# 2235854410/CCVPE

Hardware: AMD Instinct MI355X
Metric: query images/sec (VIGOR, 512x512 sat / 320x640 grd) (higher is better)
Workload: dtype f32; 1 GPU; vigor_samearea_fov360_b32; variant=vigor_ori_prior, batch_per_gpu=32, global_batch=32, parallelism=image-parallel x1, all_gather of 20 B/query results, schedule=two streams per GPU (aerial encoder + orientation decoder on the second)

## Files before the change

ccvpe_amd/csrc/kernels.h:

```cpp
#pragma once
#include <functional>
#include <vector>
#include <hip/hip_runtime.h>
#include <stdint.h>
#include "ticket.h"

namespace ccvpe {

extern thread_local unsigned long long g_launches;
#define CCVPE_LAUNCH(...) do { ++::ccvpe::g_launches; hipLaunchKernelGGL(__VA_ARGS__); } while (0)

struct LdsAttr { size_t set[16] = {0}; };
inline void ensure_dynamic_lds(LdsAttr& state, const void* kernel, size_t bytes) {
    int dev = 0;
    if (hipGetDevice(&dev) != hipSuccess || dev < 0 || dev >= 16) dev = 0;
    if (bytes > state.set[dev] && hipFuncSetAttribute(kernel, hipFuncAttributeMaxDynamicSharedMemorySize, (int)bytes) == hipSuccess) state.set[dev] = bytes;
}

enum Act { ACT_NONE = 0, ACT_RELU = 1, ACT_SWISH = 2 };

struct Dst {
    float* ptr;
    int ld;
    int coff;
    int split;
    long long plane;
};

enum { MODE_CONV = 0, MODE_DECONV = 1 };

struct ConvParams {
    const float* in;
    int in_ld;
    int B, H, W, Cin;
    int OH, OW;
    int KH, KW, stride, pad_t, pad_l;
    const float* wpk;
    const unsigned short* w_hi;
    const unsigned short* w_lo;
    int Kpad;
    int Npad;
    int nchunks;
    const float* bias;
    int N;
    int act;
    const float* gate;
    const float* resid;
    int resid_ld;
    Dst dst[3];
    int ndst;
    int mode;
    int deconv_cout;
    int M;
    unsigned in_bytes;
    int in_split;
    unsigned in_plane_bytes;
    unsigned w_plane_bytes;
    unsigned gate_bytes;
    int taps4;
    int kfull_chunks;
    int kfull_c0;
    int knc;
    int div_4t_mul;
    int div_nc_mul;
    int div_kw_mul;
    int vec_epi;
    int splitk;
    float* partial;
    size_t partial_floats;
    unsigned* tickets;
    int split_fused;
    unsigned fdw_mul, fdw_shift, fdh_mul, fdh_shift;
    const float* wino_w;
    int wino_n16;
    int wino_nb, wino_n16_off;
    unsigned wino_bytes;
    const float* wino4_w;
    unsigned wino4_bytes;
    const float* wino4x_w;
    unsigned wino4x_bytes;
    int wino4x_cfg;
    const float* proj_w;
    unsigned proj_bytes;
    const float* se_rows;
    int se_nrows, se_sq;
    float se_inv_hw;
    const float* se_b1;
    const float* se_w2;
    const float* se_b2;
};

enum { TILE_AUTO = 0 };
static constexpr int CONV_TICKETS = 8192;
static constexpr int SPLIT_FUSED = 64;
int conv_igemm_num_tiles();
double conv_igemm_tile_util(const ConvParams& p, int tile);
long long conv_igemm_tile_blocks(const ConvParams& p, int tile);
int conv_igemm_prepare(ConvParams& p);
int conv_igemm_k_index(int cin, int taps, int tap, int c);
int launch_conv_igemm(const ConvParams& p, int tile, hipStream_t s);
int conv_igemm_npad();
bool conv_igemm_tile_is_bf16x3(int tile);
bool conv_igemm_tile_can_fuse_split(int tile);
void launch_splitk_reduce(const ConvParams& p, hipStream_t s);
struct Bf16x3Tile { int bm, bn; const char* name; void (*launch)(const ConvParams&, hipStream_t); };
int bf16x3_num_tiles();
const Bf16x3Tile* bf16x3_tile(int i);
struct WinoTile { int bm, bn; const char* name; void (*launch)(const ConvParams&, hipStream_t); int f; int xcfg; };
int wino_num_tiles();
const WinoTile* wino_tile(int i);
bool conv_wino_supported(const ConvParams& p);
bool conv_wino4_supported(const ConvParams& p);
bool conv_wino_tile_supported(const ConvParams& p, int tile);
bool conv_igemm_tile_is_wino4(int tile);
void launch_wino4_64(const ConvParams& p, hipStream_t s);
void launch_wino4_128(const ConvParams& p, hipStream_t s);
bool conv_wino4_tail_applied();
bool conv_igemm_tile_is_wino4x(int tile);
int conv_igemm_tile_wino4x_cfg(int tile);
void launch_wino4x(const ConvParams& p, hipStream_t s);
bool conv_wino4x_supported(const ConvParams& p);
int conv_wino4x_config(int N);
size_t conv_wino4x_pack(int N, int cin, const std::function<float(int, int, int)>& get, std::vector<float>& out, int* cfg_out);
size_t conv_wino4_pack(int N, int cin, const std::function<float(int, int, int)>& get, std::vector<float>& out);
bool conv_igemm_tile_is_wino(int tile);
size_t conv_wino_pack(int N, int cin, const std::function<float(int, int, int)>& get, std::vector<float>& out, int* n16_out);
struct PwTile { int bm, bn; const char* name; void (*launch)(const ConvParams&, hipStream_t); int proj_rt; };
int pw_num_tiles();
const PwTile* pw_tile(int i);
bool conv_pw_supported(const ConvParams& p);
bool conv_pw_fits(int bn, int kpad);
bool conv_pw_tile_ok(int i, const ConvParams& p);
int conv_pw_tile_proj_rt(int i);
int conv_igemm_tile_proj_rt(int tile);
int conv_proj_lat_tile();
bool conv_proj_supported(const ConvParams& p, int rt);
void launch_proj(const ConvParams& p, int rt, hipStream_t s);
bool conv_proj_wanted(int N, int cin);
bool conv_proj_has(int rt, int N);
size_t conv_proj_pack(int N, int cin, const std::function<float(int, int)>& get, std::vector<float>& out, int taps = 1);
bool conv_proj_lat_wanted(int taps, int KH, int KW, int cinp);
bool conv_igemm_tile_is_pw(int tile);
bool conv_igemm_tile_is_proj(int tile);
int conv_igemm_last_tile();
const char* conv_igemm_tile_name(int tile);

struct StemParams {
    const float* in;
    int B, H, W, OH, OW;
    int pad_t, pad_l;
    int circular;
    const float* w;
    const float* bias;
    float* out;
};
void launch_stem(const StemParams& p, hipStream_t s);

struct StemDwParams {
    StemParams st;
    const float* wd;
    const float* bd;
    float* out;
    float* pool_partial;
    SeTicket se;
};
int stem_dw_tiles(int OH, int OW);
void launch_stem_dw(const StemDwParams& p, hipStream_t s);

struct DwParams {
    const float* in;
    int B, H, W, C, OH, OW;
    int k, stride, pad_t, pad_l, circular;
    const float* w;
    const float* bias;
    float* out;
    float* pool_partial;
    int S;
    SeTicket se;
};
void launch_depthwise(const DwParams& p, hipStream_t s);
int depthwise_strip_lanes(int B, int OH, int OW, int C, int k, int stride);

struct MbFrontParams {
    const float* x;
    int B, H, W, Cin, cinp;
    int mid;
    const float* we;
    const float* be;
    const float* wd;
    const float* bd;
    int k, s, pad_t, pad_l, circular, OH, OW;
    float* out;
    float* pool;
    SeTicket se;
    int spread;
};
void launch_mbconv_front(const MbFrontParams& p, hipStream_t s);
int mbconv_front_tiles(int k, int s, int OH, int OW);
int mbconv_front_ticket_rows(const MbFrontParams& p);
int mbconv_image_ticket_rows(const MbFrontParams& p);
int mbconv_front_ticket_split(const MbFrontParams& p);
bool mbconv_front_supported(int k, int s, int cin, int mid);
bool mbconv_front_profitable(int k);
bool mbconv_image_supported(const MbFrontParams& p);
int mbconv_image_strips(const MbFrontParams& p);
void launch_mbconv_image(const MbFrontParams& p, hipStream_t s);

struct SeParams {
    const float* pool_partial;
    int B, S, C, SQ;
    float inv_hw;
    const float* w1;
    const float* b1;
    const float* w2;
    const float* b2;
    float* gate;
    float* pooled;
    int SC;
    float* sq;
};
void launch_se(const SeParams& p, hipStream_t s);

struct GrdDescParams {
    const float* y;
    int B, Hf, Wf, Ntot;
    int nlev;
    int c[6], off[6];
    const float* wh[6];
    float b2[6];
    float* desc;
    int loff[6];
    int Ltot;
};
void launch_grd_desc(const GrdDescParams& p, hipStream_t s);

struct MatchParams {
    const float* x;
    int x_ld;
    int B, HW, C;
    const float* g;
    int g_ld, L;
    int R;
    int shift[32];
    uint32_t inmax;
    float* ms;
    float* cat_max;  int cat_max_ld;
    float* cat_all;  int cat_all_ld;  int rpad;
    int P;
    float* gg_scratch;
    int prep_done;
    int no_wide;
};
void launch_match(const MatchParams& p, hipStream_t s);
void launch_match_prep(const MatchParams& p, hipStream_t s);
void launch_match_prep_all(const MatchParams* ps, int n, hipStream_t s);
int match_pixels_per_block(int HW, int C);
size_t match_scratch_floats(int C);

struct TailConvParams {
    const float* in;
    int B, H, W;
    const float* w;
    float bias[2];
    int cout;
    int normalize;
    float* out;
    float* raw;
};
void launch_tail_conv(const TailConvParams& p, hipStream_t s);
// ... 138 lines not shown
```

ccvpe_amd/csrc/kernels_wino.hip:

```cpp
#include "igemm_common.h"

#include <algorithm>

namespace ccvpe {

typedef float f32x2 __attribute__((ext_vector_type(2)));

#ifndef CCVPE_WINO_SCALAR_COLUMNS
#define CCVPE_WINO_SCALAR_COLUMNS 0
#endif

template <int NW, int NM, int GC, bool FUSED = false>
__global__ __launch_bounds__(NW * NM * 64) __attribute__((amdgpu_waves_per_eu(2, 2))) void conv_wino_kernel(const ConvParams p) {
    constexpr int NT = NW * NM * 64;
    constexpr int NITEM = 256 * NM;
    constexpr int ITEMS = (NITEM + NT - 1) / NT;
    constexpr int PXS = GC * 8 + 4;
    constexpr int PROWS = 8 * NM + 2;
    constexpr int RAW_F4 = PROWS * 18 * GC * 2;
    constexpr int RAW_ITEMS = (RAW_F4 + NT - 1) / NT;
    constexpr unsigned OOB = 0x80000000u;
    constexpr bool VDB = NM == 1;
    constexpr int VSZ = 4096 * NM;

// ... 163 lines not shown
                    for (int x = 0; x < 16; ++x) Vw[x * 256 + g_lds[i]] = vi[x];
                }
            }
            __syncthreads();
            if (!VDB) {
#pragma unroll
                for (int i = 0; i < ITEMS; ++i)
                    if (NT * ITEMS == NITEM || tid + i * NT < NITEM) {
#pragma unroll
                        for (int x = 0; x < 16; ++x) Vw[x * 256 + g_lds[i]] = v[VDB ? 0 : i][x];
                    }
            }
            const bool group_end = sub == glen - 1;
            if (group_end) {
                CCVPE_WINO_STORE_RAW();
                gstart += glen;
                ++gidx;
                glen = glen_lo + (gidx < n_hi ? 1 : 0);
            }
            if (!VDB || group_end) __syncthreads();
            vbuf ^= 1;
            const unsigned wb = last_chunk ? w_base_n : w_base;
            const int chn = last_chunk ? c_begin : ch + 1;
            __builtin_amdgcn_sched_barrier(0);
            f32x2 fa[2][2][2];
#define CCVPE_WINO_FRAGS(buf, g)                                                                         \
    _Pragma("unroll") for (int e = 0; e < 2; ++e) {                                                      \
        fa[buf][e][0] = *reinterpret_cast<const f32x2*>(va + ((g) * 2 + e) * 256);                       \
        fa[buf][e][1] = *reinterpret_cast<const f32x2*>(va + ((g) * 2 + e) * 256 + 128);                 \
    }
            CCVPE_WINO_FRAGS(0, 0);
#pragma unroll
            for (int g = 0; g < 8; ++g) {
                const int cur = g & 1;
                if (g + 1 < 8) { CCVPE_WINO_FRAGS(cur ^ 1, g + 1); }
                __builtin_amdgcn_sched_barrier(0);
#pragma unroll
                for (int e = 0; e < 2; ++e) {
                    const int x = g * 2 + e;
                    acc[x][0] = __builtin_amdgcn_mfma_f32_16x16x4f32(bq[x].x, fa[cur][e][0].x, acc[x][0], 0, 0, 0);
                    acc[x][1] = __builtin_amdgcn_mfma_f32_16x16x4f32(bq[x].x, fa[cur][e][1].x, acc[x][1], 0, 0, 0);
                    acc[x][0] = __builtin_amdgcn_mfma_f32_16x16x4f32(bq[x].y, fa[cur][e][0].y, acc[x][0], 0, 0, 0);
                    acc[x][1] = __builtin_amdgcn_mfma_f32_16x16x4f32(bq[x].y, fa[cur][e][1].y, acc[x][1], 0, 0, 0);
                }
                __builtin_amdgcn_sched_barrier(0);
                CCVPE_WINO_LOAD_B(wb, chn, g);
            }
#undef CCVPE_WINO_FRAGS
            __builtin_amdgcn_sched_barrier(0);
        }

        {
            const int n = (nb * NW + wave) * 16 + 4 * (lane >> 4);
            f32x4 bias = {0.f, 0.f, 0.f, 0.f};
            if (!split) {
#pragma unroll
                for (int i = 0; i < 4; ++i) bias[i] = n + i < p.N ? p.bias[n + i] : 0.f;
            }
            const float lo = act == ACT_RELU ? 0.f : -__builtin_inff();
            const size_t pix0 = ((size_t)b * p.H + (size_t)(by * NM + wset) * 8) * p.W + (size_t)bx * 16;
            float* obase = split ? p.partial + ((size_t)blockIdx.z * p.M + pix0) * p.N : p.dst[0].ptr + pix0 * ld + p.dst[0].coff;
            const __amdgpu_buffer_rsrc_t o_rsrc = __builtin_amdgcn_make_buffer_rsrc(obase, 0, 0x7fffffff, 0x00020000);
            const int tl = lane & 15;
            const unsigned o_lane = n < p.N ? (unsigned)((((tl >> 3) * 2 * p.W + (tl & 7) * 2) * ld + n) * 4) : OOB;
#pragma unroll
            for (int h = 0; h < 2; ++h) {
                f32x4 tt[2][4];
#pragma unroll
                for (int c = 0; c < 4; ++c) {
                    tt[0][c] = acc[0 * 4 + c][h] + acc[1 * 4 + c][h] + acc[2 * 4 + c][h];
                    tt[1][c] = acc[1 * 4 + c][h] - acc[2 * 4 + c][h] - acc[3 * 4 + c][h];
                }
#pragma unroll
                for (int a = 0; a < 2; ++a) {
                    f32x4 y[2];
                    y[0] = tt[a][0] + tt[a][1] + tt[a][2] + bias;
                    y[1] = tt[a][1] - tt[a][2] - tt[a][3] + bias;
#pragma unroll
                    for (int dx = 0; dx < 2; ++dx) {
                        f32x4 v;
#pragma unroll
                        for (int i = 0; i < 4; ++i) v[i] = y[dx][i] < lo ? lo : y[dx][i];
                        const int soff = (((h * 4 + a) * p.W + dx) * ld) * 4;
                        __builtin_amdgcn_raw_buffer_store_b128(__builtin_bit_cast(__attribute__((__vector_size__(4 * sizeof(unsigned)))) unsigned, v), o_rsrc, o_lane, soff, FUSED ? 16 : 0);
                        __builtin_amdgcn_sched_barrier(0);
                        asm volatile("s_nop 1");
                        __builtin_amdgcn_sched_barrier(0);
                    }
                }
            }
        }
        if (FUSED) {
            if (splitk_ticket(p, item, reinterpret_cast<unsigned*>(Vs))) fin_mask |= 1ull << ordinal;
        }
        if (FUSED) ++ordinal;
        if (!have_n) break;
#pragma unroll
        for (int x = 0; x < 16; ++x) {
            acc[x][0] = f32x4{0.f, 0.f, 0.f, 0.f};
            acc[x][1] = f32x4{0.f, 0.f, 0.f, 0.f};
        }
        item = item_n; nb = nb_n; b = b_n; by = by_n; bx = bx_n; w_base = w_base_n;
    }
    while (FUSED && fin_mask) {
        const int k = __builtin_ctzll(fin_mask);
        fin_mask &= fin_mask - 1;
        int nb_f, b_f, by_f, bx_f;
        CCVPE_WINO_DECODE(item_first + k * stride, nb_f, b_f, by_f, bx_f);
        splitk_finish<NT>(p, (b_f * p.H + by_f * NM * 8) * p.W + bx_f * 16, 8 * NM, 16, p.W, nb_f * NW * 16, NW * 16);
    }
#undef CCVPE_WINO_LOAD_RAW
#undef CCVPE_WINO_STORE_RAW
#undef CCVPE_WINO_LOAD_B
#undef CCVPE_WINO_ROFF
#undef CCVPE_WINO_DECODE
#undef CCVPE_WINO_WBASE
}

template <int NW, int NM, int GC>
static void launch_wino(const ConvParams& p_in, hipStream_t s) {
    ConvParams p = p_in;
    if (p.splitk > 1) {
        const int nch = p.Cin >> 3;
        const int per = (nch + p.splitk - 1) / p.splitk;
        p.splitk = (nch + per - 1) / per;
    }
    constexpr size_t lds = (4096 * NM * (NM == 1 ? 2 : 1) + (8 * NM + 2) * 18 * (GC * 8 + 4)) * sizeof(float);
    static_assert(2 * lds <= 160 * 1024, "two workgroups per CU");
    static LdsAttr attr, attr_f;
    const int mblocks = p.B * (p.W >> 4) * (p.H / (8 * NM));
    const int nblocks = (p.wino_n16 + NW - 1) / NW;
    const int resident = 2 * 256 / (p.splitk > 1 ? p.splitk : 1);
    dim3 grid(std::min(mblocks * nblocks, std::max(resident, 8)), 1, p.splitk > 1 ? p.splitk : 1);
    if (p.splitk <= 1 || p.tickets == nullptr || mblocks * nblocks > CONV_TICKETS || (mblocks * nblocks + (int)grid.x - 1) / (int)grid.x + 1 > 64) p.split_fused = 0;
    if (p.split_fused) {
        auto kern = conv_wino_kernel<NW, NM, GC, true>;
        ensure_dynamic_lds(attr_f, reinterpret_cast<const void*>(kern), lds);
        CCVPE_LAUNCH(kern, grid, dim3(NW * NM * 64), lds, s, p);
        return;
    }
    auto kern = conv_wino_kernel<NW, NM, GC, false>;
    ensure_dynamic_lds(attr, reinterpret_cast<const void*>(kern), lds);
    CCVPE_LAUNCH(kern, grid, dim3(NW * NM * 64), lds, s, p);
    if (p.splitk > 1) launch_splitk_reduce(p, s);
}

static const WinoTile WINO_TILES[] = {
    {256, 32, "conv_wino_64x32", launch_wino<2, 2, 2>, 2, -1},
    {128, 48, "conv_wino_32x48", launch_wino<3, 1, 2>, 2, -1},
    {128, 64, "conv_wino_32x64", launch_wino<4, 1, 4>, 2, -1},
    {128, 80, "conv_wino_32x80", launch_wino<5, 1, 4>, 2, -1},
    {256, 48, "conv_wino_64x48", launch_wino<3, 2, 2>, 2, -1},
    {256, 64, "conv_wino4_16x64", launch_wino4_64, 4, -1},
    {256, 128, "conv_wino4_16x128", launch_wino4_128, 4, -1},
    {256, 32, "conv_wino4x_32", launch_wino4x, 4, 0},
    {256, 48, "conv_wino4x_48", launch_wino4x, 4, 1},
    {256, 64, "conv_wino4x_64", launch_wino4x, 4, 2},
    {256, 80, "conv_wino4x_80", launch_wino4x, 4, 3},
    {256, 96, "conv_wino4x_96", launch_wino4x, 4, 4},
    {256, 128, "conv_wino4x_128", launch_wino4x, 4, 5},
};
int wino_num_tiles() { return (int)(sizeof(WINO_TILES) / sizeof(WINO_TILES[0])); }
const WinoTile* wino_tile(int i) { return &WINO_TILES[i]; }

bool conv_wino_supported(const ConvParams& p) {
    return p.wino_w != nullptr && p.KH == 3 && p.KW == 3 && p.stride == 1 && p.pad_t == 1 && p.pad_l == 1 && p.mode == MODE_CONV &&
           p.gate == nullptr && p.resid == nullptr && p.ndst == 1 && !p.dst[0].split && !p.in_split && p.OH == p.H && p.OW == p.W &&
           p.W % 16 == 0 && p.H % 16 == 0 && p.Cin % 8 == 0 && p.N % 4 == 0 && p.dst[0].ld % 4 == 0 && p.dst[0].coff % 4 == 0;
}

size_t conv_wino_pack(int N, int cin, const std::function<float(int, int, int)>& get, std::vector<float>& out, int* n16_out) {
    static const double G[4][3] = {{1.0, 0.0, 0.0}, {0.5, 0.5, 0.5}, {0.5, -0.5, 0.5}, {0.0, 0.0, 1.0}};
    const int n16 = (N + 15) / 16;
    const int nch = cin / 8;
    out.assign((size_t)nch * 16 * n16 * 128, 0.f);
    for (int n = 0; n < N; ++n)
        for (int c = 0; c < cin; ++c) {
            double g[3][3], tmp[4][3];
            for (int i = 0; i < 3; ++i)
                for (int j = 0; j < 3; ++j) g[i][j] = (double)get(n, i * 3 + j, c);
            for (int r = 0; r < 4; ++r)
                for (int j = 0; j < 3; ++j) tmp[r][j] = G[r][0] * g[0][j] + G[r][1] * g[1][j] + G[r][2] * g[2][j];
            const int chunk = c / 8, k = c % 8;
            for (int r = 0; r < 4; ++r)
                for (int q = 0; q < 4; ++q) {
                    const double uv = tmp[r][0] * G[q][0] + tmp[r][1] * G[q][1] + tmp[r][2] * G[q][2];
                    const int xi = r * 4 + q;
                    const size_t idx = ((((size_t)chunk * 8 + xi / 2) * n16 + n / 16) * 64 + (k & 3) * 16 + (n % 16)) * 4 + (xi & 1) * 2 + (k >> 2);
                    out[idx] = (float)uv;
                }
        }
    *n16_out = n16;
    return out.size();
}

}
```

ccvpe_amd/csrc/kernels_wino4.hip:

```cpp
#include "igemm_common.h"

#include <algorithm>
#include <thread>
#include <type_traits>

namespace ccvpe {

typedef float f32x2 __attribute__((ext_vector_type(2)));

static constexpr int W4_PITCH = 20;
static constexpr int W4_PLANE = 385;
static constexpr int W4_GCH = 16;
static constexpr int W4_VFLOATS = 4 * 18 * 64 * 2;
static constexpr int W4_RAW_F4 = 18 * 18 * 4;

__device__ __forceinline__ void w4_bt(const float d0, const float d1, const float d2, const float d3, const float d4, const float d5,
                                      float& t0, float& t1, float& t2, float& t3, float& t4, float& t5) {
    const float a = fmaf(-4.f, d2, d4), b = fmaf(-4.f, d1, d3);
    const float c = d4 - d2, e = d3 - d1;
    t0 = fmaf(4.f, d0, fmaf(-5.f, d2, d4));
    t1 = a + b;
    t2 = a - b;
    t3 = fmaf(2.f, e, c);
    t4 = fmaf(-2.f, e, c);
    t5 = fmaf(4.f, d1, fmaf(-5.f, d3, d5));
}
__device__ __forceinline__ void w4_at(const float m0, const float m1, const float m2, const float m3, const float m4, const float m5,
                                      float& y0, float& y1, float& y2, float& y3) {
    const float s1 = m1 + m2, d1 = m1 - m2, s2 = m3 + m4, d2 = m3 - m4;
    y0 = m0 + s1 + s2;
    y1 = fmaf(2.f, d2, d1);
    y2 = fmaf(4.f, s2, s1);
    y3 = fmaf(8.f, d2, d1) + m5;
}

template <int NW, bool FUSED = false>
__global__ __launch_bounds__(NW * 64) __attribute__((amdgpu_waves_per_eu(2, 2))) void conv_wino4_kernel(const ConvParams p) {
    static_assert(NW == 4 || NW == 8, "waves w and w + 4 share the k-step w & 3 of a 16-channel group");
    constexpr int NT = NW * 64;
    constexpr int RAW_ITEMS = NW == 4 ? 6 : 3;
    constexpr int RAW_HALVES = RAW_ITEMS / 3;
    constexpr unsigned OOB = 0x80000000u;

    extern __shared__ __attribute__((aligned(16))) float smem[];
    float* Vs = smem;
    float* Rs = smem + W4_VFLOATS;

    const int tid = threadIdx.x;
    const int lane = tid & 63;
    const int wave = tid >> 6;

    const int mbx = p.W >> 4, mby = p.H >> 4;
    const int mblocks = p.B * mbx * mby;
    const int total = mblocks * (p.wino_nb ? p.wino_nb : (p.wino_n16 + NW - 1) / NW);

    const int xcd = blockIdx.x & 7;
    const int stride = ((int)gridDim.x >> 3) + (xcd < ((int)gridDim.x & 7) ? 1 : 0);
    const int S = p.splitk > 1 ? p.splitk : 1;
    const int item_begin = xcd * (total >> 3) + min(xcd, total & 7);
    const int item_end = item_begin + (total >> 3) + (xcd < (total & 7) ? 1 : 0);
    int item = item_begin + ((int)blockIdx.x >> 3);
    if (item >= item_end) return;
    const int item_first = item;
    int ordinal = 0;
    unsigned long long fin_mask = 0;

    const __amdgpu_buffer_rsrc_t in_rsrc = __builtin_amdgcn_make_buffer_rsrc(const_cast<float*>(p.in), 0, p.in_bytes, 0x00020000);
    const __amdgpu_buffer_rsrc_t w_rsrc = __builtin_amdgcn_make_buffer_rsrc(const_cast<float*>(p.wino4_w), 0, p.wino4_bytes, 0x00020000);

    int nb, b, by, bx;
    const int z = (int)blockIdx.z;
#define CCVPE_W4_DECODE(it_, nb_, b_, by_, bx_)                                                          \
    {                                                                                                    \
        nb_ = (it_) / mblocks;                                                                           \
        const int mb_ = (it_) - nb_ * mblocks;                                                           \
        b_ = mb_ / (mbx * mby);                                                                          \
        const int rem_ = mb_ - b_ * (mbx * mby);                                                         \
        by_ = rem_ / mbx;                                                                                \
        bx_ = rem_ - by_ * mbx;                                                                          \
    }
    CCVPE_W4_DECODE(item, nb, b, by, bx);

    unsigned r_off[RAW_ITEMS];
    const int r_ch = (tid & 3) * 4;
    const int r_px0 = tid >> 2;
#define CCVPE_W4_ROFF(b_, by_, bx_, live_)                                                               \
    _Pragma("unroll") for (int i = 0; i < RAW_ITEMS; ++i) {                                              \
        int j = tid + i * NT;                                                                            \
        asm volatile("" : "+v"(j));    \
        const int px = j >> 2, q = j & 3;                                                                \
        const int py = px / 18, pxx = px - py * 18;                                                      \
        const int y = (by_) * 16 - 1 + py, x = (bx_) * 16 - 1 + pxx;                                     \
        const bool ok = (live_) && j < W4_RAW_F4 && (unsigned)y < (unsigned)p.H && (unsigned)x < (unsigned)p.W; \
        r_off[i] = ok ? (unsigned)(((((b_) * p.H + y) * p.W + x) * p.in_ld + q * 4) * 4) : OOB;          \
    }
    CCVPE_W4_ROFF(b, by, bx, true);

    const int tk = lane & 3, ttx = (lane >> 2) & 3, tty = lane >> 4;
    const int tks = wave & 3;
    const float* t_src = Rs + (4 * tks + tk) * W4_PLANE + (4 * tty) * W4_PITCH + 4 * ttx;
    float* t_dst = Vs + ((tks * 18) * 64 + tk * 16 + tty * 4 + ttx) * 2;

    const unsigned w_quad_b = (unsigned)p.wino_n16 * 1024u;
    const unsigned w_step_b = w_quad_b * 9u;
#define CCVPE_W4_WBASE(nb_) ((nb_) * NW + wave + p.wino_n16_off < p.wino_n16 ? (unsigned)((nb_) * NW + wave + p.wino_n16_off) * 1024u + (unsigned)lane * 16u : OOB)
    unsigned w_base = CCVPE_W4_WBASE(nb);

    const int ngr_all = (p.Cin + W4_GCH - 1) / W4_GCH;
    const int g_per = (ngr_all + S - 1) / S;
    const int g_begin = min(z * g_per, ngr_all), g_end = min(g_begin + g_per, ngr_all);
    if (g_begin >= g_end) return;
    const int tail_ks = (p.Cin - (ngr_all - 1) * W4_GCH + 3) >> 2;

    f32x4 raw[3];
    float bq[36];
#define CCVPE_W4_LOAD_RAW(c0, half)                                        \
    _Pragma("unroll") for (int i = 0; i < 3; ++i) {                                                    \
        const unsigned o_ = ((c0) + r_ch < p.Cin) ? r_off[3 * (half) + i] : OOB;                         \
        raw[i] = __builtin_bit_cast(f32x4, __builtin_amdgcn_raw_buffer_load_b128(in_rsrc, o_, (c0) * 4, 0)); \
    }
#define CCVPE_W4_STORE_RAW(half)                                                                         \
    _Pragma("unroll") for (int i = 0; i < 3; ++i) {                                                    \
        const int px_ = r_px0 + (NT / 4) * (3 * (half) + i);                                             \
        if (px_ < 18 * 18) {                                                                             \
            const int py_ = (px_ * 3641) >> 16;                          \
            float* d_ = Rs + r_ch * W4_PLANE + py_ * W4_PITCH + (px_ - py_ * 18);                        \
            d_[0] = raw[i].x; d_[W4_PLANE] = raw[i].y; d_[2 * W4_PLANE] = raw[i].z; d_[3 * W4_PLANE] = raw[i].w; \
        }                                                                                                \
    }
#define CCVPE_W4_LOAD_B(wb, ks, qd)              \
    {                                                                                                    \
        const f32x4 t4_ = __builtin_bit_cast(f32x4, __builtin_amdgcn_raw_buffer_load_b128(w_rsrc, wb, (ks) * w_step_b + (qd) * w_quad_b, 0)); \
        bq[4 * (qd)] = t4_.x; bq[4 * (qd) + 1] = t4_.y; bq[4 * (qd) + 2] = t4_.z; bq[4 * (qd) + 3] = t4_.w; \
    }

    f32x4 acc[36];
#pragma unroll
    for (int x = 0; x < 36; ++x) acc[x] = f32x4{0.f, 0.f, 0.f, 0.f};

    CCVPE_W4_LOAD_RAW(g_begin * W4_GCH, 0);
#pragma unroll
    for (int qd = 0; qd < 9; ++qd) { CCVPE_W4_LOAD_B(w_base, g_begin * 4, qd); }
    CCVPE_W4_STORE_RAW(0);
    if (RAW_HALVES == 2) {
        CCVPE_W4_LOAD_RAW(g_begin * W4_GCH, 1);
        CCVPE_W4_STORE_RAW(1);
    }
    __syncthreads();

    const float* va0 = Vs + lane * 2;
    const bool split = p.splitk > 1;
    const int ld = split ? p.N : p.dst[0].ld;
    const int act = split ? ACT_NONE : p.act;

    while (true) {
        const int item_n = item + stride;
        const bool have_n = item_n < item_end;
        int nb_n, b_n, by_n, bx_n;
        CCVPE_W4_DECODE(have_n ? item_n : item, nb_n, b_n, by_n, bx_n);
        const unsigned w_base_n = have_n ? CCVPE_W4_WBASE(nb_n) : OOB;

        for (int g = g_begin; g < g_end; ++g) {
            const bool last_group = g == g_end - 1;
            const int nks = g == ngr_all - 1 ? tail_ks : 4;
            auto half_item = [&](auto hfc) {
                constexpr int HF = decltype(hfc)::value;
                float t[3][6];
                float dc[2][6];
#pragma unroll
                for (int r = 0; r < 6; ++r) dc[0][r] = t_src[r * W4_PITCH];
#pragma unroll
                for (int c = 0; c < 6; ++c) {
                    if (c + 1 < 6) {
#pragma unroll
                        for (int r = 0; r < 6; ++r) dc[(c + 1) & 1][r] = t_src[r * W4_PITCH + c + 1];
                    }
                    float u0, u1, u2, u3, u4, u5;
                    w4_bt(dc[c & 1][0], dc[c & 1][1], dc[c & 1][2], dc[c & 1][3], dc[c & 1][4], dc[c & 1][5], u0, u1, u2, u3, u4, u5);
                    t[0][c] = HF ? u3 : u0; t[1][c] = HF ? u4 : u1; t[2][c] = HF ? u5 : u2;
                }
#pragma unroll
                for (int ii = 0; ii < 3; ++ii) {
                    float v0, v1, v2, v3, v4, v5;
                    w4_bt(t[ii][0], t[ii][1], t[ii][2], t[ii][3], t[ii][4], t[ii][5], v0, v1, v2, v3, v4, v5);
                    float* td = t_dst + HF * (9 * 128) + ii * (3 * 128);
                    *reinterpret_cast<f32x2*>(td) = f32x2{v0, v1};
                    *reinterpret_cast<f32x2*>(td + 128) = f32x2{v2, v3};
                    *reinterpret_cast<f32x2*>(td + 256) = f32x2{v4, v5};
                }
            };
            if (tks >= nks) {
            } else if (NW == 4) {
                half_item(std::integral_constant<int, 0>{});
                half_item(std::integral_constant<int, 1>{});
            } else if (wave < 4) {
                half_item(std::integral_constant<int, 0>{});
            } else {
                half_item(std::integral_constant<int, 1>{});
            }
            __syncthreads();
            const int c0n = last_group ? g_begin * W4_GCH : (g + 1) * W4_GCH;
            if (last_group) { CCVPE_W4_ROFF(b_n, by_n, bx_n, have_n); }
            CCVPE_W4_LOAD_RAW(c0n, 0);
            __builtin_amdgcn_sched_barrier(0);
#pragma unroll 1
            for (int ks = 0; ks < nks; ++ks) {
                const bool last_step = last_group && ks == nks - 1;
                const unsigned wb = last_step ? w_base_n : w_base;
                const int ksn = last_step ? g_begin * 4 : g * 4 + ks + 1;
                const float* va = va0 + ks * (18 * 128);
                f32x2 fa[3];
                fa[0] = *reinterpret_cast<const f32x2*>(va);
                fa[1] = *reinterpret_cast<const f32x2*>(va + 128);
#pragma unroll
                for (int xp = 0; xp < 18; ++xp) {
                    if (xp + 2 < 18) fa[(xp + 2) % 3] = *reinterpret_cast<const f32x2*>(va + (xp + 2) * 128);
                    __builtin_amdgcn_sched_barrier(0);
                    acc[2 * xp] = __builtin_amdgcn_mfma_f32_16x16x4f32(bq[2 * xp], fa[xp % 3].x, acc[2 * xp], 0, 0, 0);
                    acc[2 * xp + 1] = __builtin_amdgcn_mfma_f32_16x16x4f32(bq[2 * xp + 1], fa[xp % 3].y, acc[2 * xp + 1], 0, 0, 0);
                    if (xp & 1) {
                        __builtin_amdgcn_sched_barrier(0);
                        CCVPE_W4_LOAD_B(wb, ksn, xp >> 1);
                    }
                }
                __builtin_amdgcn_sched_barrier(0);
                if (RAW_HALVES == 2 && ks == 1) {
                    CCVPE_W4_STORE_RAW(0);
                    CCVPE_W4_LOAD_RAW(c0n, 1);
                    __builtin_amdgcn_sched_barrier(0);
                }
            }
            CCVPE_W4_STORE_RAW(RAW_HALVES - 1);
            __syncthreads();
        }

        {
            const int n = (nb * NW + wave) * 16 + 4 * (lane >> 4);
            const bool nok = n < p.N;
            const f32x4 bias = (split || !nok) ? f32x4{0.f, 0.f, 0.f, 0.f} : *reinterpret_cast<const f32x4*>(p.bias + n);
            const float lo = act == ACT_RELU ? 0.f : -__builtin_inff();
            const size_t pix0 = ((size_t)b * p.H + (size_t)by * 16) * p.W + (size_t)bx * 16;
            float* obase = split ? p.partial + ((size_t)z * p.M + pix0) * p.N : p.dst[0].ptr + pix0 * ld + p.dst[0].coff;
            const __amdgpu_buffer_rsrc_t o_rsrc = __builtin_amdgcn_make_buffer_rsrc(obase, 0, 0x7fffffff, 0x00020000);
            const int oty = (lane >> 2) & 3, otx = lane & 3;
            const unsigned o_lane = nok ? (unsigned)((((oty * 4) * p.W + otx * 4) * ld + n) * 4) : OOB;
#pragma unroll
            for (int i = 0; i < 4; ++i) {
                float tt[4][6];
#pragma unroll
                for (int q = 0; q < 6; ++q)
                    w4_at(acc[0 * 6 + q][i], acc[1 * 6 + q][i], acc[2 * 6 + q][i], acc[3 * 6 + q][i], acc[4 * 6 + q][i], acc[5 * 6 + q][i],
                          tt[0][q], tt[1][q], tt[2][q], tt[3][q]);
#pragma unroll
                for (int a = 0; a < 4; ++a) {
                    float yy[4];
                    w4_at(tt[a][0], tt[a][1], tt[a][2], tt[a][3], tt[a][4], tt[a][5], yy[0], yy[1], yy[2], yy[3]);
#pragma unroll
                    for (int c = 0; c < 4; ++c) acc[4 * a + c][i] = yy[c];
                }
            }
#pragma unroll
            for (int a = 0; a < 4; ++a)
#pragma unroll
                for (int c = 0; c < 4; ++c) {
                    f32x4 v;
#pragma unroll
                    for (int i = 0; i < 4; ++i) {
                        const float t = acc[4 * a + c][i] + bias[i];
                        v[i] = t < lo ? lo : t;
                    }
                    const int soff = ((a * p.W + c) * ld) * 4;
                    __builtin_amdgcn_raw_buffer_store_b128(__builtin_bit_cast(__attribute__((__vector_size__(4 * sizeof(unsigned)))) unsigned, v), o_rsrc, o_lane, soff, FUSED ? 16 : 0);
                    __builtin_amdgcn_sched_barrier(0);
                    asm volatile("s_nop 1");
                    __builtin_amdgcn_sched_barrier(0);
                }
        }
        if (FUSED) {
            if (splitk_ticket(p, nb * mblocks + (b * mby + by) * mbx + bx, reinterpret_cast<unsigned*>(Vs))) fin_mask |= 1ull << ordinal;
        }
        if (FUSED) ++ordinal;
        if (!have_n) break;
#pragma unroll
        for (int x = 0; x < 36; ++x) acc[x] = f32x4{0.f, 0.f, 0.f, 0.f};
        item = item_n; nb = nb_n; b = b_n; by = by_n; bx = bx_n; w_base = w_base_n;
    }
    while (FUSED && fin_mask) {
        const int k = __builtin_ctzll(fin_mask);
        fin_mask &= fin_mask - 1;
        int nb_f, b_f, by_f, bx_f;
        CCVPE_W4_DECODE(item_first + k * stride, nb_f, b_f, by_f, bx_f);
        splitk_finish<NT>(p, (b_f * p.H + by_f * 16) * p.W + bx_f * 16, 16, 16, p.W, nb_f * NW * 16, NW * 16);
    }
#undef CCVPE_W4_DECODE
#undef CCVPE_W4_ROFF
#undef CCVPE_W4_WBASE
#undef CCVPE_W4_LOAD_RAW
#undef CCVPE_W4_STORE_RAW
#undef CCVPE_W4_LOAD_B
}

template <int NW>
static void launch_wino4_plain(const ConvParams& p_in, hipStream_t s) {
    ConvParams p = p_in;
    if (p.splitk > 1) {
        const int ngr = (p.Cin + W4_GCH - 1) / W4_GCH;
        const int per = (ngr + p.splitk - 1) / p.splitk;
        p.splitk = (ngr + per - 1) / per;
    }
    constexpr size_t lds = (W4_VFLOATS + W4_GCH * W4_PLANE) * sizeof(float);
    static_assert(2 * lds <= 160 * 1024, "two workgroups per CU");
    static LdsAttr attr, attr_f;
    const int mblocks = p.B * (p.W >> 4) * (p.H >> 4);
    const int nblocks = p.wino_nb ? p.wino_nb : (p.wino_n16 + NW - 1) / NW;
    const int S = p.splitk > 1 ? p.splitk : 1;
    const int resident = (NW == 4 ? 2 : 1) * 256 / S;
    dim3 grid(std::min(mblocks * nblocks, std::max(resident, 8)), 1, S);
    const int per_wg = (mblocks * nblocks + (int)grid.x - 1) / (int)grid.x + 8;
    if (S <= 1 || p.tickets == nullptr || mblocks * nblocks > CONV_TICKETS || per_wg > 64) p.split_fused = 0;
    const dim3 block(NW * 64);
    if (p.split_fused) { auto kern = conv_wino4_kernel<NW, true>; ensure_dynamic_lds(attr_f, reinterpret_cast<const void*>(kern), lds); CCVPE_LAUNCH(kern, grid, block, lds, s, p); return; }
    auto kern = conv_wino4_kernel<NW, false>;
    ensure_dynamic_lds(attr, reinterpret_cast<const void*>(kern), lds);
    CCVPE_LAUNCH(kern, grid, block, lds, s, p);
    if (S > 1) launch_splitk_reduce(p, s);
}

static thread_local bool g_tail_applied = false;
bool conv_wino4_tail_applied() { return g_tail_applied; }

template <int NW>
static void launch_wino4(const ConvParams& p, hipStream_t s) {
    g_tail_applied = false;
    if (p.splitk != 255) { launch_wino4_plain<NW>(p, s); return; }
    ConvParams a = p;
    a.splitk = 1;
    const int mblocks = p.B * (p.W >> 4) * (p.H >> 4);
    const int nblocks = (p.wino_n16 + NW - 1) / NW;
    const int resident = (NW == 4 ? 2 : 1) * 256;
    const int rem = (mblocks * nblocks) % resident;
    const int ngr = (p.Cin + W4_GCH - 1) / W4_GCH;
    const int tail_nb = mblocks > 0 ? rem / mblocks : 0;
    int split = tail_nb > 0 ? std::min(resident / rem, ngr / 2) : 0;
    const int n0 = (nblocks - tail_nb) * NW * 16;
    if (rem == 0 || rem % mblocks != 0 || tail_nb >= nblocks || split < 2 || p.partial == nullptr ||
        (size_t)split * p.M * (size_t)(p.N - n0) > p.partial_floats || (n0 & 3) != 0) {
        launch_wino4_plain<NW>(a, s);
        return;
    }
    g_tail_applied = true;
    a.wino_nb = nblocks - tail_nb; a.split_fused = 0;
    launch_wino4_plain<NW>(a, s);
    ConvParams b = p;
    b.wino_nb = tail_nb; b.wino_n16_off = (nblocks - tail_nb) * NW;
    b.N = p.N - n0; b.bias = p.bias + n0; b.dst[0].coff = p.dst[0].coff + n0;
    b.splitk = split;
    launch_wino4_plain<NW>(b, s);
}

void launch_wino4_64(const ConvParams& p, hipStream_t s) { launch_wino4<4>(p, s); }
void launch_wino4_128(const ConvParams& p, hipStream_t s) { launch_wino4<8>(p, s); }

bool conv_wino4_supported(const ConvParams& p) {
    return p.wino4_w != nullptr && p.KH == 3 && p.KW == 3 && p.stride == 1 && p.pad_t == 1 && p.pad_l == 1 && p.mode == MODE_CONV &&
           p.gate == nullptr && p.resid == nullptr && p.ndst == 1 && !p.dst[0].split && !p.in_split && p.OH == p.H && p.OW == p.W &&
           p.W % 16 == 0 && p.H % 16 == 0 && p.Cin % 8 == 0 && p.N % 4 == 0 && p.dst[0].ld % 4 == 0 && p.dst[0].coff % 4 == 0;
}

size_t conv_wino4_pack(int N, int cin, const std::function<float(int, int, int)>& get, std::vector<float>& out) {
    static const double G[6][3] = {{0.25, 0.0, 0.0}, {-1.0 / 6, -1.0 / 6, -1.0 / 6}, {-1.0 / 6, 1.0 / 6, -1.0 / 6},
                                   {1.0 / 24, 1.0 / 12, 1.0 / 6}, {1.0 / 24, -1.0 / 12, 1.0 / 6}, {0.0, 0.0, 1.0}};
    const int n16 = (N + 15) / 16;
    const int ksteps = ((cin + 15) / 16) * 4;
    out.assign((size_t)ksteps * 9 * n16 * 256, 0.f);
    auto work = [&](int n_lo, int n_hi) {
        for (int n = n_lo; n < n_hi; ++n)
            for (int c = 0; c < cin; ++c) {
                double g[3][3], tmp[6][3];
                for (int i = 0; i < 3; ++i)
                    for (int j = 0; j < 3; ++j) g[i][j] = (double)get(n, i * 3 + j, c);
                for (int r = 0; r < 6; ++r)
                    for (int j = 0; j < 3; ++j) tmp[r][j] = G[r][0] * g[0][j] + G[r][1] * g[1][j] + G[r][2] * g[2][j];
                const int ks = c / 4, k = c % 4;
                for (int r = 0; r < 6; ++r)
                    for (int q = 0; q < 6; ++q) {
                        const double uv = tmp[r][0] * G[q][0] + tmp[r][1] * G[q][1] + tmp[r][2] * G[q][2];
                        const int xi = r * 6 + q;
                        const size_t idx = ((((size_t)ks * 9 + xi / 4) * n16 + n / 16) * 64 + k * 16 + (n % 16)) * 4 + (xi & 3);
                        out[idx] = (float)uv;
                    }
            }
    };
    const int nthreads = std::max(1, std::min(16, (int)std::thread::hardware_concurrency()));
    if (nthreads == 1 || (long long)N * cin < 4096) { work(0, N); return out.size(); }
    std::vector<std::thread> th;
    for (int t = 0; t < nthreads; ++t) th.emplace_back(work, (int)((long long)N * t / nthreads), (int)((long long)N * (t + 1) / nthreads));
    for (auto& x : th) x.join();
    return out.size();
}

}
```

Baseline: 2546 queries/s.

## Double-buffer Winograd F(4,3) input transform to overlap with GEMM in 128-wide tile

Adds a double-buffered variant of the 512-thread Winograd F(4,3) kernel. It keeps two raw-input and two transformed-V LDS buffers, so the input transform for the next channel group overlaps the multiply for the current one, and half the waves transform before the GEMM and half after. This removes one barrier-bounded serial transform phase per group but doubles LDS use. It also XOR-swizzles the V store and load slots to reduce LDS bank conflicts, and adds optional s_memtime phase instrumentation behind a compile flag. The existing wino4_16x128 tile now points to the double-buffered launcher, and the old single-buffer kernel stays available as a new 's' tile entry.

```diff
diff --git a/ccvpe_amd/csrc/kernels.h b/ccvpe_amd/csrc/kernels.h
--- a/ccvpe_amd/csrc/kernels.h
+++ b/ccvpe_amd/csrc/kernels.h
@@ -115,6 +115,7 @@
 bool conv_igemm_tile_is_wino4(int tile);
 void launch_wino4_64(const ConvParams& p, hipStream_t s);
 void launch_wino4_128(const ConvParams& p, hipStream_t s);
+void launch_wino4_128d(const ConvParams& p, hipStream_t s);
 bool conv_wino4_tail_applied();
 bool conv_igemm_tile_is_wino4x(int tile);
 int conv_igemm_tile_wino4x_cfg(int tile);
diff --git a/ccvpe_amd/csrc/kernels_wino.hip b/ccvpe_amd/csrc/kernels_wino.hip
--- a/ccvpe_amd/csrc/kernels_wino.hip
+++ b/ccvpe_amd/csrc/kernels_wino.hip
@@ -339,13 +339,14 @@
     {128, 80, "conv_wino_32x80", launch_wino<5, 1, 4>, 2, -1},
     {256, 48, "conv_wino_64x48", launch_wino<3, 2, 2>, 2, -1},
     {256, 64, "conv_wino4_16x64", launch_wino4_64, 4, -1},
-    {256, 128, "conv_wino4_16x128", launch_wino4_128, 4, -1},
+    {256, 128, "conv_wino4_16x128", launch_wino4_128d, 4, -1},
     {256, 32, "conv_wino4x_32", launch_wino4x, 4, 0},
     {256, 48, "conv_wino4x_48", launch_wino4x, 4, 1},
     {256, 64, "conv_wino4x_64", launch_wino4x, 4, 2},
     {256, 80, "conv_wino4x_80", launch_wino4x, 4, 3},
     {256, 96, "conv_wino4x_96", launch_wino4x, 4, 4},
     {256, 128, "conv_wino4x_128", launch_wino4x, 4, 5},
+    {256, 128, "conv_wino4_16x128s", launch_wino4_128, 4, -1},
 };
 int wino_num_tiles() { return (int)(sizeof(WINO_TILES) / sizeof(WINO_TILES[0])); }
 const WinoTile* wino_tile(int i) { return &WINO_TILES[i]; }
diff --git a/ccvpe_amd/csrc/kernels_wino4.hip b/ccvpe_amd/csrc/kernels_wino4.hip
--- a/ccvpe_amd/csrc/kernels_wino4.hip
+++ b/ccvpe_amd/csrc/kernels_wino4.hip
@@ -13,6 +13,22 @@
 static constexpr int W4_GCH = 16;
 static constexpr int W4_VFLOATS = 4 * 18 * 64 * 2;
 static constexpr int W4_RAW_F4 = 18 * 18 * 4;
+static constexpr int W4_RFLOATS = W4_GCH * W4_PLANE;
+
+#ifndef CCVPE_W4_CLOCK
+#define CCVPE_W4_CLOCK 0
+#endif
+#if CCVPE_W4_CLOCK
+__device__ unsigned long long g_w4_stamps[1024 * 2 * 8];
+#define CCVPE_W4_STAMP(ph_)                                       \
+    {                                                             \
+        const unsigned long long t_ = __builtin_amdgcn_s_memtime(); \
+        clk[ph_] += t_ - clk_last;                                \
+        clk_last = t_;                                            \
+    }
+#else
+#define CCVPE_W4_STAMP(ph_)
+#endif
 
 __device__ __forceinline__ void w4_bt(const float d0, const float d1, const float d2, const float d3, const float d4, const float d5,
                                       float& t0, float& t1, float& t2, float& t3, float& t4, float& t5) {
@@ -34,9 +50,14 @@
     y3 = fmaf(8.f, d2, d1) + m5;
 }
 
-template <int NW, bool FUSED = false>
+template <int NW, bool FUSED = false, bool DB = false>
 __global__ __launch_bounds__(NW * 64) __attribute__((amdgpu_waves_per_eu(2, 2))) void conv_wino4_kernel(const ConvParams p) {
     static_assert(NW == 4 || NW == 8, "waves w and w + 4 share the k-step w & 3 of a 16-channel group");
+    static_assert(!DB || NW == 8, "double-buffered: one 512-thread workgroup per CU");
+#if CCVPE_W4_CLOCK
+    unsigned long long clk[4] = {0, 0, 0, 0};
+    unsigned long long clk_last = __builtin_amdgcn_s_memtime();
+#endif
     constexpr int NT = NW * 64;
     constexpr int RAW_ITEMS = NW == 4 ? 6 : 3;
     constexpr int RAW_HALVES = RAW_ITEMS / 3;
@@ -44,7 +65,8 @@
 
     extern __shared__ __attribute__((aligned(16))) float smem[];
     float* Vs = smem;
-    float* Rs = smem + W4_VFLOATS;
+    float* Rs = smem + (DB ? 2 : 1) * W4_VFLOATS;
+    unsigned* const flag = reinterpret_cast<unsigned*>(DB ? Rs + 2 * W4_RFLOATS : Vs);
 
     const int tid = threadIdx.x;
     const int lane = tid & 63;
@@ -99,7 +121,7 @@
     const int tk = lane & 3, ttx = (lane >> 2) & 3, tty = lane >> 4;
     const int tks = wave & 3;
     const float* t_src = Rs + (4 * tks + tk) * W4_PLANE + (4 * tty) * W4_PITCH + 4 * ttx;
-    float* t_dst = Vs + ((tks * 18) * 64 + tk * 16 + tty * 4 + ttx) * 2;
+    float* t_dst = Vs + ((tks * 18) * 64 + tk * 16 + (tty ^ tk) * 4 + ttx) * 2;
 
     const unsigned w_quad_b = (unsigned)p.wino_n16 * 1024u;
     const unsigned w_step_b = w_quad_b * 9u;
@@ -119,12 +141,12 @@
         const unsigned o_ = ((c0) + r_ch < p.Cin) ? r_off[3 * (half) + i] : OOB;                         \
         raw[i] = __builtin_bit_cast(f32x4, __builtin_amdgcn_raw_buffer_load_b128(in_rsrc, o_, (c0) * 4, 0)); \
     }
-#define CCVPE_W4_STORE_RAW(half)                                                                         \
+#define CCVPE_W4_STORE_RAW(rb, half)                                                                     \
     _Pragma("unroll") for (int i = 0; i < 3; ++i) {                                                    \
         const int px_ = r_px0 + (NT / 4) * (3 * (half) + i);                                             \
         if (px_ < 18 * 18) {                                                                             \
             const int py_ = (px_ * 3641) >> 16;                          \
-            float* d_ = Rs + r_ch * W4_PLANE + py_ * W4_PITCH + (px_ - py_ * 18);                        \
+            float* d_ = (rb) + r_ch * W4_PLANE + py_ * W4_PITCH + (px_ - py_ * 18);                      \
             d_[0] = raw[i].x; d_[W4_PLANE] = raw[i].y; d_[2 * W4_PLANE] = raw[i].z; d_[3 * W4_PLANE] = raw[i].w; \
         }                                                                                                \
     }
@@ -138,20 +160,59 @@
 #pragma unroll
     for (int x = 0; x < 36; ++x) acc[x] = f32x4{0.f, 0.f, 0.f, 0.f};
 
+    auto half_item = [&](auto hfc, const int ro, const int vo) {
+        constexpr int HF = decltype(hfc)::value;
+        const float* src = t_src + ro;
+        float t[3][6];
+        float dc[2][6];
+#pragma unroll
+        for (int r = 0; r < 6; ++r) dc[0][r] = src[r * W4_PITCH];
+#pragma unroll
+        for (int c = 0; c < 6; ++c) {
+            if (c + 1 < 6) {
+#pragma unroll
+                for (int r = 0; r < 6; ++r) dc[(c + 1) & 1][r] = src[r * W4_PITCH + c + 1];
+            }
+            float u0, u1, u2, u3, u4, u5;
+            w4_bt(dc[c & 1][0], dc[c & 1][1], dc[c & 1][2], dc[c & 1][3], dc[c & 1][4], dc[c & 1][5], u0, u1, u2, u3, u4, u5);
+            t[0][c] = HF ? u3 : u0; t[1][c] = HF ? u4 : u1; t[2][c] = HF ? u5 : u2;
+        }
+#pragma unroll
+        for (int ii = 0; ii < 3; ++ii) {
+            float v0, v1, v2, v3, v4, v5;
+            w4_bt(t[ii][0], t[ii][1], t[ii][2], t[ii][3], t[ii][4], t[ii][5], v0, v1, v2, v3, v4, v5);
+            float* td = t_dst + vo + HF * (9 * 128) + ii * (3 * 128);
+            *reinterpret_cast<f32x2*>(td) = f32x2{v0, v1};
+            *reinterpret_cast<f32x2*>(td + 128) = f32x2{v2, v3};
+            *reinterpret_cast<f32x2*>(td + 256) = f32x2{v4, v5};
+        }
+    };
+
     CCVPE_W4_LOAD_RAW(g_begin * W4_GCH, 0);
 #pragma unroll
     for (int qd = 0; qd < 9; ++qd) { CCVPE_W4_LOAD_B(w_base, g_begin * 4, qd); }
-    CCVPE_W4_STORE_RAW(0);
+    CCVPE_W4_STORE_RAW(Rs, 0);
     if (RAW_HALVES == 2) {
         CCVPE_W4_LOAD_RAW(g_begin * W4_GCH, 1);
-        CCVPE_W4_STORE_RAW(1);
+        CCVPE_W4_STORE_RAW(Rs, 1);
+    }
+    if (DB) {
+        CCVPE_W4_LOAD_RAW((g_begin + 1) * W4_GCH, 0);
+        CCVPE_W4_STORE_RAW(Rs + W4_RFLOATS, 0);
+        __syncthreads();
+        if (tks < (g_begin == ngr_all - 1 ? tail_ks : 4)) {
+            if (wave < 4) half_item(std::integral_constant<int, 0>{}, 0, 0);
+            else half_item(std::integral_constant<int, 1>{}, 0, 0);
+        }
     }
     __syncthreads();
 
-    const float* va0 = Vs + lane * 2;
+    const int vslot = lane ^ (((lane >> 4) & 3) << 2);
+    const float* va0 = Vs + vslot * 2;
     const bool split = p.splitk > 1;
     const int ld = split ? p.N : p.dst[0].ld;
     const int act = split ? ACT_NONE : p.act;
+    int par = 0;
 
     while (true) {
         const int item_n = item + stride;
@@ -163,44 +224,33 @@
         for (int g = g_begin; g < g_end; ++g) {
             const bool last_group = g == g_end - 1;
             const int nks = g == ngr_all - 1 ? tail_ks : 4;
-            auto half_item = [&](auto hfc) {
-                constexpr int HF = decltype(hfc)::value;
-                float t[3][6];
-                float dc[2][6];
-#pragma unroll
-                for (int r = 0; r < 6; ++r) dc[0][r] = t_src[r * W4_PITCH];
-#pragma unroll
-                for (int c = 0; c < 6; ++c) {
-                    if (c + 1 < 6) {
-#pragma unroll
-                        for (int r = 0; r < 6; ++r) dc[(c + 1) & 1][r] = t_src[r * W4_PITCH + c + 1];
-                    }
-                    float u0, u1, u2, u3, u4, u5;
-                    w4_bt(dc[c & 1][0], dc[c & 1][1], dc[c & 1][2], dc[c & 1][3], dc[c & 1][4], dc[c & 1][5], u0, u1, u2, u3, u4, u5);
-                    t[0][c] = HF ? u3 : u0; t[1][c] = HF ? u4 : u1; t[2][c] = HF ? u5 : u2;
+            int c0n;
+            bool tr1 = false;
+            int r1 = 0, v1 = 0;
+            if (DB) {
+                const int g1 = last_group ? g_begin : g + 1;
+                tr1 = (!last_group || have_n) && tks < (g1 == ngr_all - 1 ? tail_ks : 4);
+                c0n = (g + 2 < g_end ? g + 2 : g_begin + (g + 2 - g_end)) * W4_GCH;
+                if (g + 2 == g_end) { CCVPE_W4_ROFF(b_n, by_n, bx_n, have_n); }
+                r1 = (par ^ 1) * W4_RFLOATS;
+                v1 = (par ^ 1) * W4_VFLOATS;
+                if (wave < 4 && tr1) half_item(std::integral_constant<int, 0>{}, r1, v1);
+                CCVPE_W4_STAMP(0);
+            } else {
+                if (tks >= nks) {
+                } else if (NW == 4) {
+                    half_item(std::integral_constant<int, 0>{}, 0, 0);
+                    half_item(std::integral_constant<int, 1>{}, 0, 0);
+                } else if (wave < 4) {
+                    half_item(std::integral_constant<int, 0>{}, 0, 0);
+                } else {
+                    half_item(std::integral_constant<int, 1>{}, 0, 0);
                 }
-#pragma unroll
-                for (int ii = 0; ii < 3; ++ii) {
-                    float v0, v1, v2, v3, v4, v5;
-                    w4_bt(t[ii][0], t[ii][1], t[ii][2], t[ii][3], t[ii][4], t[ii][5], v0, v1, v2, v3, v4, v5);
-                    float* td = t_dst + HF * (9 * 128) + ii * (3 * 128);
-                    *reinterpret_cast<f32x2*>(td) = f32x2{v0, v1};
-                    *reinterpret_cast<f32x2*>(td + 128) = f32x2{v2, v3};
-                    *reinterpret_cast<f32x2*>(td + 256) = f32x2{v4, v5};
-                }
-            };
-            if (tks >= nks) {
-            } else if (NW == 4) {
-                half_item(std::integral_constant<int, 0>{});
-                half_item(std::integral_constant<int, 1>{});
-            } else if (wave < 4) {
-                half_item(std::integral_constant<int, 0>{});
-            } else {
-                half_item(std::integral_constant<int, 1>{});
-            }
-            __syncthreads();
-            const int c0n = last_group ? g_begin * W4_GCH : (g + 1) * W4_GCH;
-            if (last_group) { CCVPE_W4_ROFF(b_n, by_n, bx_n, have_n); }
+                __syncthreads();
+                CCVPE_W4_STAMP(0);
+                c0n = last_group ? g_begin * W4_GCH : (g + 1) * W4_GCH;
+                if (last_group) { CCVPE_W4_ROFF(b_n, by_n, bx_n, have_n); }
+            }
             CCVPE_W4_LOAD_RAW(c0n, 0);
             __builtin_amdgcn_sched_barrier(0);
 #pragma unroll 1
@@ -208,7 +258,7 @@
                 const bool last_step = last_group && ks == nks - 1;
                 const unsigned wb = last_step ? w_base_n : w_base;
                 const int ksn = last_step ? g_begin * 4 : g * 4 + ks + 1;
-                const float* va = va0 + ks * (18 * 128);
+                const float* va = va0 + (DB ? par * W4_VFLOATS : 0) + ks * (18 * 128);
                 f32x2 fa[3];
                 fa[0] = *reinterpret_cast<const f32x2*>(va);
                 fa[1] = *reinterpret_cast<const f32x2*>(va + 128);
@@ -225,13 +275,20 @@
                 }
                 __builtin_amdgcn_sched_barrier(0);
                 if (RAW_HALVES == 2 && ks == 1) {
-                    CCVPE_W4_STORE_RAW(0);
+                    CCVPE_W4_STORE_RAW(Rs, 0);
                     CCVPE_W4_LOAD_RAW(c0n, 1);
                     __builtin_amdgcn_sched_barrier(0);
                 }
             }
-            CCVPE_W4_STORE_RAW(RAW_HALVES - 1);
+            CCVPE_W4_STORE_RAW(DB ? Rs + par * W4_RFLOATS : Rs, RAW_HALVES - 1);
+            CCVPE_W4_STAMP(1);
+            if (DB && wave >= 4 && tr1) {
+                half_item(std::integral_constant<int, 1>{}, r1, v1);
+                CCVPE_W4_STAMP(0);
+            }
             __syncthreads();
+            CCVPE_W4_STAMP(2);
+            par ^= 1;
         }
 
         {
@@ -277,9 +334,10 @@
                 }
         }
         if (FUSED) {
-            if (splitk_ticket(p, nb * mblocks + (b * mby + by) * mbx + bx, reinterpret_cast<unsigned*>(Vs))) fin_mask |= 1ull << ordinal;
+            if (splitk_ticket(p, nb * mblocks + (b * mby + by) * mbx + bx, flag)) fin_mask |= 1ull << ordinal;
         }
         if (FUSED) ++ordinal;
+        CCVPE_W4_STAMP(3);
         if (!have_n) break;
 #pragma unroll
         for (int x = 0; x < 36; ++x) acc[x] = f32x4{0.f, 0.f, 0.f, 0.f};
@@ -292,6 +350,13 @@
         CCVPE_W4_DECODE(item_first + k * stride, nb_f, b_f, by_f, bx_f);
         splitk_finish<NT>(p, (b_f * p.H + by_f * 16) * p.W + bx_f * 16, 16, 16, p.W, nb_f * NW * 16, NW * 16);
     }
+#if CCVPE_W4_CLOCK
+    if (lane == 0 && (wave & 3) == 0 && blockIdx.x < 1024 && blockIdx.z == 0) {
+        unsigned long long* st = g_w4_stamps + (blockIdx.x * 2 + (wave >> 2)) * 8;
+        for (int i = 0; i < 4; ++i) st[i] = clk[i];
+        st[4] = 1;
+    }
+#endif
 #undef CCVPE_W4_DECODE
 #undef CCVPE_W4_ROFF
 #undef CCVPE_W4_WBASE
@@ -299,40 +364,65 @@
 #undef CCVPE_W4_STORE_RAW
 #undef CCVPE_W4_LOAD_B
 }
-
-template <int NW>
+#undef CCVPE_W4_STAMP
+
+template <int NW, bool DB>
 static void launch_wino4_plain(const ConvParams& p_in, hipStream_t s) {
     ConvParams p = p_in;
+    const int ngr = (p.Cin + W4_GCH - 1) / W4_GCH;
     if (p.splitk > 1) {
-        const int ngr = (p.Cin + W4_GCH - 1) / W4_GCH;
         const int per = (ngr + p.splitk - 1) / p.splitk;
         p.splitk = (ngr + per - 1) / per;
     }
-    constexpr size_t lds = (W4_VFLOATS + W4_GCH * W4_PLANE) * sizeof(float);
-    static_assert(2 * lds <= 160 * 1024, "two workgroups per CU");
+    const int S = p.splitk > 1 ? p.splitk : 1;
+    if (DB && (ngr + S - 1) / S < 2) { launch_wino4_plain<NW, false>(p, s); return; }
+    constexpr size_t lds = (DB ? 2 : 1) * (W4_VFLOATS + W4_RFLOATS) * sizeof(float) + (DB ? 16 : 0);
+    static_assert((NW == 4 ? 2 : 1) * lds <= 160 * 1024, "two 256-thread workgroups per CU, or one 512-thread workgroup");
     static LdsAttr attr, attr_f;
     const int mblocks = p.B * (p.W >> 4) * (p.H >> 4);
     const int nblocks = p.wino_nb ? p.wino_nb : (p.wino_n16 + NW - 1) / NW;
-    const int S = p.splitk > 1 ? p.splitk : 1;
     const int resident = (NW == 4 ? 2 : 1) * 256 / S;
     dim3 grid(std::min(mblocks * nblocks, std::max(resident, 8)), 1, S);
     const int per_wg = (mblocks * nblocks + (int)grid.x - 1) / (int)grid.x + 8;
     if (S <= 1 || p.tickets == nullptr || mblocks * nblocks > CONV_TICKETS || per_wg > 64) p.split_fused = 0;
     const dim3 block(NW * 64);
-    if (p.split_fused) { auto kern = conv_wino4_kernel<NW, true>; ensure_dynamic_lds(attr_f, reinterpret_cast<const void*>(kern), lds); CCVPE_LAUNCH(kern, grid, block, lds, s, p); return; }
-    auto kern = conv_wino4_kernel<NW, false>;
-    ensure_dynamic_lds(attr, reinterpret_cast<const void*>(kern), lds);
-    CCVPE_LAUNCH(kern, grid, block, lds, s, p);
+    if (p.split_fused) { auto kern = conv_wino4_kernel<NW, true, DB>; ensure_dynamic_lds(attr_f, reinterpret_cast<const void*>(kern), lds); CCVPE_LAUNCH(kern, grid, block, lds, s, p); }
+    else {
+        auto kern = conv_wino4_kernel<NW, false, DB>;
+        ensure_dynamic_lds(attr, reinterpret_cast<const void*>(kern), lds);
+        CCVPE_LAUNCH(kern, grid, block, lds, s, p);
+    }
+#if CCVPE_W4_CLOCK
+    {
+        (void)hipStreamSynchronize(s);
+        std::vector<unsigned long long> h(1024 * 2 * 8);
+        (void)hipMemcpyFromSymbol(h.data(), HIP_SYMBOL(g_w4_stamps), h.size() * 8);
+        double sum[2][4] = {};
+        int n = 0;
+        for (unsigned i = 0; i < grid.x && i < 1024; ++i) {
+            if (!h[(i * 2) * 8 + 4]) continue;
+            ++n;
+            for (int w = 0; w < 2; ++w)
+                for (int k = 0; k < 4; ++k) sum[w][k] += (double)h[(i * 2 + w) * 8 + k];
+        }
+        if (n) std::fprintf(stderr, "w4clock NW %d DB %d B %d H %d W %d Cin %d N %d nb %d S %d fused %d | wave0 T %.0f M %.0f B %.0f E %.0f | wave4 T %.0f M %.0f B %.0f E %.0f | wgs %d\n",
+                            NW, (int)DB, p.B, p.H, p.W, p.Cin, p.N, nblocks, S, (int)p.split_fused, sum[0][0] / n, sum[0][1] / n, sum[0][2] / n, sum[0][3] / n,
+                            sum[1][0] / n, sum[1][1] / n, sum[1][2] / n, sum[1][3] / n, n);
+        std::vector<unsigned long long> z(h.size(), 0);
+        (void)hipMemcpyToSymbol(HIP_SYMBOL(g_w4_stamps), z.data(), z.size() * 8);
+    }
+#endif
+    if (p.split_fused) return;
     if (S > 1) launch_splitk_reduce(p, s);
 }
 
 static thread_local bool g_tail_applied = false;
 bool conv_wino4_tail_applied() { return g_tail_applied; }
 
-template <int NW>
+template <int NW, bool DB = false>
 static void launch_wino4(const ConvParams& p, hipStream_t s) {
     g_tail_applied = false;
-    if (p.splitk != 255) { launch_wino4_plain<NW>(p, s); return; }
+    if (p.splitk != 255) { launch_wino4_plain<NW, DB>(p, s); return; }
     ConvParams a = p;
     a.splitk = 1;
     const int mblocks = p.B * (p.W >> 4) * (p.H >> 4);
@@ -345,21 +435,22 @@
     const int n0 = (nblocks - tail_nb) * NW * 16;
     if (rem == 0 || rem % mblocks != 0 || tail_nb >= nblocks || split < 2 || p.partial == nullptr ||
         (size_t)split * p.M * (size_t)(p.N - n0) > p.partial_floats || (n0 & 3) != 0) {
-        launch_wino4_plain<NW>(a, s);
+        launch_wino4_plain<NW, DB>(a, s);
         return;
     }
     g_tail_applied = true;
     a.wino_nb = nblocks - tail_nb; a.split_fused = 0;
-    launch_wino4_plain<NW>(a, s);
+    launch_wino4_plain<NW, DB>(a, s);
     ConvParams b = p;
     b.wino_nb = tail_nb; b.wino_n16_off = (nblocks - tail_nb) * NW;
     b.N = p.N - n0; b.bias = p.bias + n0; b.dst[0].coff = p.dst[0].coff + n0;
     b.splitk = split;
-    launch_wino4_plain<NW>(b, s);
+    launch_wino4_plain<NW, DB>(b, s);
 }
 
 void launch_wino4_64(const ConvParams& p, hipStream_t s) { launch_wino4<4>(p, s); }
 void launch_wino4_128(const ConvParams& p, hipStream_t s) { launch_wino4<8>(p, s); }
+void launch_wino4_128d(const ConvParams& p, hipStream_t s) { launch_wino4<8, true>(p, s); }
 
 bool conv_wino4_supported(const ConvParams& p) {
     return p.wino4_w != nullptr && p.KH == 3 && p.KW == 3 && p.stride == 1 && p.pad_t == 1 && p.pad_l == 1 && p.mode == MODE_CONV &&
```

New measurement: 2576 queries/s, median of 6. 1.01x the previous value.
